# YuanchenBei/ColdRec

Hardware: AMD Instinct MI355X
Metric: ranked items/sec (full-catalogue eval) (higher is better)
Workload: dtype f32; 1 GPU; configs[3] full-catalogue eval: 1000000-row user table x 10000000 items, d=128, k=20, f32 tables, user block 131072 per step, rated CSR (mean ~50) + 20% cold-item bitmap ('warm' setting), item table row-sharded over 1 GPU(s); items=10000000, dim=128, k=20, parallelism=single GPU

## Files before the change

### coldrec_amd/_lib.py

```python
from __future__ import annotations

import ctypes
import os
import subprocess

_HERE = os.path.dirname(os.path.abspath(__file__))
LIB_PATH = os.environ.get("CRH_LIB") or os.path.join(_HERE, "lib", "libcoldrec_hip.so")
CSRC = os.path.join(_HERE, "csrc")

PAD_IDX = 0x7FFFFFFF
MASKED_SCORE = -1.0e9
MAX_K = 128

_lib = None

_vp, _i32, _i64, _sz, _f32 = ctypes.c_void_p, ctypes.c_int, ctypes.c_int64, ctypes.c_size_t, ctypes.c_float
_f64 = ctypes.c_double

SIGNATURES = {
    "crh_last_error": (ctypes.c_char_p, []),
    "crh_version": (_i32, []),
    "crh_score_topk_supports_dim": (_i32, [_i32]),
    "crh_score_topk_workspace_bytes": (_sz, [_i64, _i64, _i32, _i32]),
    "crh_score_topk_min_workspace_bytes": (_sz, [_i64, _i32]),
    "crh_score_topk_route": (_i32, [_i32, _i64, _i64, _i32, _i32, _sz, _i32, _i32, _vp, _vp]),
    "crh_score_topk_route_kernel": (ctypes.c_char_p, [_i32]),
    "crh_score_topk_screened": (_i32, [_i32, _i64, _i64, _i32, _i32, _sz, _i32, _i32]),
    "crh_score_topk_uncertified": (_i64, [_vp, _vp]),
    "crh_score_topk_screen_plan": (_i32, [_i64, _i64, _sz, _i32, _vp, _vp]),
    "crh_score_topk_screen_ordered": (_i32, [_i64, _i64, _sz, _i32]),
    "crh_score_topk_screen_map": (_i32, [_vp, _vp, _i64, _i64, _i64, _i32, _vp, _vp, _vp, _vp]),
    "crh_score_topk_f32": (_i32, [_vp, _vp, _i64, _vp, _i64, _i32, _vp, _vp, _vp, _i32, _i64, _vp, _vp,
                                  _vp, _sz, _vp]),
    "crh_score_topk_f32_ex": (_i32, [_vp, _vp, _i64, _vp, _i64, _i32, _vp, _vp, _vp, _i32, _i64, _vp, _vp,
                                     _vp, _sz, _vp, _i32, _vp, _vp]),
    "crh_score_topk_f16_supports_dim": (_i32, [_i32]),
    "crh_score_topk_f16_workspace_bytes": (_sz, [_i64, _i64, _i32, _i32]),
    "crh_score_topk_f16_ex": (_i32, [_vp, _vp, _i64, _vp, _i64, _i32, _vp, _vp, _vp, _i32, _i64, _vp, _vp,
                                     _vp, _sz, _vp, _i32, _vp, _vp]),
    "crh_mask_topk_f32": (_i32, [_vp, _i64, _i64, _i64, _vp, _vp, _vp, _i32, _i64, _i32, _vp, _vp, _vp]),
    "crh_merge_topk": (_i32, [_vp, _vp, _i32, _i64, _i32, _i32, _vp, _vp, _vp]),
    "crh_bpr_workspace_bytes": (_sz, [_i64]),
    "crh_bpr_plan_ints": (_i64, [_i64]),
    "crh_bpr_heavy_threshold": (_i32, []),
    "crh_bpr_plan_build_host": (_i32, [_vp, _vp, _vp, _i64, _i64, _vp]),
    "crh_bpr_plan_build": (_i32, [_vp, _vp, _vp, _i64, _i64, _vp, _vp]),
    "crh_bpr_plan_build_large_workspace_bytes": (_sz, [_i64, _i64]),
    "crh_bpr_plan_build_large": (_i32, [_vp, _vp, _vp, _i64, _i64, _vp, _vp, _sz, _vp]),
    "crh_bpr_fwd_bwd_f32": (_i32, [_vp, _vp, _vp, _i32, _vp, _vp, _vp, _i64, _f32, _vp, _vp, _vp, _vp, _vp, _vp,
                                   _sz, _vp]),
# ... 125 lines not shown
```

### coldrec_amd/csrc/score_screen.hip

```cpp
#include <math.h>

#include "score_topk_common.h"

#include <hipcub/device/device_radix_sort.hpp>

namespace crh_score {
namespace {

constexpr int SD = 128;
constexpr int FB_SCRATCH_SLICES = 64;

__device__ __forceinline__ float up_float(double x) {
    if (!(x <= 3.0e38)) return __builtin_inff();
    float f = (float)x;
    if ((double)f < x) f = __uint_as_float(__float_as_uint(f) + 1u);
    return f;
}

__device__ __forceinline__ int scale_exp(const unsigned* stats, int word) {
    const float m = __uint_as_float(stats[word]);
    if (!(m > 0.0f) || !(m <= 3.4e38f)) return 0;
    int E;
    frexpf(m, &E);
    return 15 - E;
// ... 453 lines not shown
    hipLaunchKernelGGL(screen_sortkey_kernel, dim3((unsigned)((n_slots + 255) / 256)), dim3(256), 0, st, idmap, ord->rowkeys, n_live,
                       item_base, n_slots, ord->skeys_in);
    CRH_HIP(hipGetLastError());
    size_t need = 0;
    CRH_HIP(hipcub::DeviceRadixSort::SortPairs(nullptr, need, ord->skeys_in, ord->skeys_out, idmap, ord->idmap, (int)n_slots, 0, 16, st));
    if (need > ord->sort_tmp_bytes) {
        crh_set_error("screened route: the ordered map's sort asks for %zu bytes of temporary storage, %zu are reserved", need,
                      ord->sort_tmp_bytes);
        return CRH_ERR_WS;
    }
    need = ord->sort_tmp_bytes;
    CRH_HIP(hipcub::DeviceRadixSort::SortPairs(ord->sort_tmp, need, ord->skeys_in, ord->skeys_out, idmap, ord->idmap, (int)n_slots, 0, 16, st));
    return CRH_OK;
}

int launch_screen_prep(const ScreenArgs& s, _Float16* packed, _Float16* uh, int64_t prefix, int32_t* idmap, unsigned* scan,
                       const ScreenOrder* ord, hipStream_t st) {
    const int64_t T = (s.n_items + 31) / 32;
    if (ord != nullptr)
        hipLaunchKernelGGL(screen_maxabs_kernel<true>, dim3(2048), dim3(256), 0, st, s.item_emb, nullptr, s.n_items, s.stats, 0, ord->rowkeys);
    else
        hipLaunchKernelGGL(screen_maxabs_kernel<false>, dim3(2048), dim3(256), 0, st, s.item_emb, nullptr, s.n_items, s.stats, 0, nullptr);
    CRH_HIP(hipGetLastError());
    hipLaunchKernelGGL(screen_maxabs_kernel<false>, dim3(256), dim3(256), 0, st, s.user_emb, s.users, s.n_users, s.stats, 1, nullptr);
    CRH_HIP(hipGetLastError());
    if (idmap != nullptr) {
        const int rc = launch_screen_map(s.bitmap, s.item_base, s.n_items, prefix, s.stats + SCREEN_STAT_LIVE, scan, idmap, ord, st);
        if (rc != CRH_OK) return rc;
        if (ord != nullptr) idmap = ord->idmap;
    }
    hipLaunchKernelGGL(screen_items_kernel, dim3((unsigned)(T < 4096 ? T : 4096)), dim3(256), 0, st, s.item_emb, s.n_items, s.bitmap,
                       s.item_base, packed, s.stats, prefix, idmap);
    CRH_HIP(hipGetLastError());
    const int64_t ub = (s.n_users * 16 + 255) / 256;
    hipLaunchKernelGGL(screen_users_kernel, dim3((unsigned)(ub < 2048 ? ub : 2048)), dim3(256), 0, st, s.user_emb, s.users, s.n_users,
                       uh, s.ustat, s.stats);
    CRH_HIP(hipGetLastError());
    return CRH_OK;
}

int screen_map_only(const uint32_t* bitmap, const float* item_emb, int64_t n_items, int64_t item_base, int64_t prefix, int ordered,
                    int32_t* map_out, int32_t* keys_out, int64_t* count, hipStream_t st) {
    auto al = [](size_t x) { return (x + 255) & ~(size_t)255; };
    const int64_t n_main = n_items - prefix, n_slots = screen_map_slots(n_main);
    const size_t o_scan = 256, o_map = o_scan + al(screen_scan_bytes(n_main)), o_rk = o_map + al((size_t)n_slots * 4),
                 o_k0 = o_rk + al((size_t)n_items * 2), o_k1 = o_k0 + al((size_t)n_slots * 2), o_m1 = o_k1 + al((size_t)n_slots * 2),
                 o_tmp = o_m1 + al((size_t)n_slots * 4), total = o_tmp + screen_sort_bytes(n_slots);
// ... 48 lines not shown
```

### coldrec_amd/csrc/score_topk.hip

```cpp
#include <math.h>
#include <stdarg.h>
#include <stdlib.h>

#include <algorithm>
#include <vector>

#include "score_topk_common.h"

using namespace crh_score;

namespace {

__device__ __forceinline__ bool pack_row_masked(const uint32_t* bitmap, int64_t gid) {
    return bitmap != nullptr && ((bitmap[gid >> 5] >> (gid & 31)) & 1u);
}

template <int D>
__global__ __launch_bounds__(256) void pack_items_kernel(const float* __restrict__ v, int64_t n_items,
                                                         float* __restrict__ packed, const uint32_t* __restrict__ bitmap,
                                                         int64_t item_base) {
    constexpr int NCH = D / 8;
    __shared__ float tile[32][D + 4];
    const int64_t t = blockIdx.x;
    for (int e = threadIdx.x; e < 32 * (D / 4); e += 256) {
// ... 810 lines not shown
    if (mode >= 2) return true;
    if (n_items < FP32_DMA_FLAG_MAX_ITEMS) return false;
    int64_t P = seed_route(esz, n_users, n_items, d);
    size_t ws = workspace_bytes;
    if (P > 0) {
        const size_t sb = seed_bytes(n_users, k);
        const size_t stage1 = dense_block_bytes(n_users, P) + packed_bytes(P, d, esz);
        const size_t stage2 = lists_bytes(n_users, k) + packed_bytes(n_items - P, d, esz);
        if (workspace_bytes >= sb + std::max(stage1, stage2)) ws = workspace_bytes - sb;
        else P = 0;
    }
    const RoutePlan r = plan_route(esz, n_users, n_items - P, d, k, true, ws, has_bitmap, 0, P > 0);
    return !r.dense && r.use_dma && r.dma_mode == 3;
}

int score_topk_screened(const float* user_emb, const int32_t* users, int64_t n_users, const float* item_emb, int64_t n_items,
                        const int64_t* rated_rowptr, const int32_t* rated_col, const uint32_t* cand_bitmap, int k, int64_t item_base,
                        float* out_score, int32_t* out_idx, void* workspace, size_t workspace_bytes, void* stream,
                        void* ev_kernel_start, void* ev_kernel_stop, const char* who);

int score_topk_any(int esz, const void* user_emb, const int32_t* users, int64_t n_users, const void* item_emb,
                   int64_t n_items, int d, const int64_t* rated_rowptr, const int32_t* rated_col,
                   const uint32_t* cand_bitmap, int k, int64_t item_base, float* out_score, int32_t* out_idx,
                   void* workspace, size_t workspace_bytes, void* stream, int n_splits, void* ev_kernel_start,
                   void* ev_kernel_stop, const char* who) {
    if (user_emb && item_emb && out_score && out_idx && workspace &&
        screen_route(esz, n_users, n_items, d, k, workspace_bytes, cand_bitmap != nullptr, n_splits))
        return score_topk_screened(reinterpret_cast<const float*>(user_emb), users, n_users, reinterpret_cast<const float*>(item_emb),
                                   n_items, rated_rowptr, rated_col, cand_bitmap, k, item_base, out_score, out_idx, workspace,
                                   workspace_bytes, stream, ev_kernel_start, ev_kernel_stop, who);
    const int64_t P = n_splits == 0 ? seed_route(esz, n_users, n_items, d) : 0;
    if (P > 0 && user_emb && item_emb && out_score && out_idx && n_users > 0 && k >= 1 && k <= CRH_MAX_K && workspace) {
        const size_t sb = seed_bytes(n_users, k);
        const size_t stage1 = dense_block_bytes(n_users, P) + packed_bytes(P, d, esz);
        const size_t stage2 = lists_bytes(n_users, k) + packed_bytes(n_items - P, d, esz);
        if (workspace_bytes >= sb + std::max(stage1, stage2)) {
            float* seed_s = reinterpret_cast<float*>(workspace);
            int32_t* seed_i = reinterpret_cast<int32_t*>(seed_s + (size_t)n_users * k);
            void* ws2 = reinterpret_cast<char*>(workspace) + sb;
            hipStream_t st = reinterpret_cast<hipStream_t>(stream);
            if (ev_kernel_start) CRH_HIP(hipEventRecord(reinterpret_cast<hipEvent_t>(ev_kernel_start), st));
            int rc = score_topk_impl(esz, user_emb, users, n_users, item_emb, P, d, rated_rowptr, rated_col, cand_bitmap, k,
                                     item_base, seed_s, seed_i, ws2, workspace_bytes - sb, stream, 0, nullptr, nullptr, who,
                                     nullptr, nullptr);
            if (rc != CRH_OK) return rc;
// ... 264 lines not shown
#ifdef CRH_PROFILE
    if (timing && use_dma) {
        rc = dma_timing_report(a, esz, d, st);
        if (rc != CRH_OK) return rc;
    }
    if (timing && !use_wg) {
        const int trc = print_wave_timing(a.wave_clock, n_waves, timing, st);
        if (trc != CRH_OK) return trc;
    }
#endif
    if (a.n_splits > 1)
        return crh_merge_topk(a.out_score, a.out_idx, a.n_splits, n_users, k, k, out_score, out_idx, stream);
    return CRH_OK;
}

int score_topk_screened(const float* user_emb, const int32_t* users, int64_t n_users, const float* item_emb, int64_t n_items,
                        const int64_t* rated_rowptr, const int32_t* rated_col, const uint32_t* cand_bitmap, int k, int64_t item_base,
                        float* out_score, int32_t* out_idx, void* workspace, size_t workspace_bytes, void* stream,
                        void* ev_kernel_start, void* ev_kernel_stop, const char* who) {
    CRH_CHECK_ARG(((uintptr_t)user_emb & 15) == 0 && ((uintptr_t)item_emb & 15) == 0, "%s: tables must be 16-byte aligned", who);
    CRH_CHECK_ARG(rated_rowptr != nullptr || rated_col == nullptr, "%s: rated_col given without rated_rowptr", who);
    CRH_CHECK_ARG(item_base >= 0 && item_base + n_items < (int64_t)CRH_PAD_IDX, "%s: item ids exceed int32", who);
    constexpr int KP = SCREEN_KP, D = 128;
    const int64_t P = screen_prefix(n_items);
    const bool compact = screen_compact(n_users, n_items, workspace_bytes, cand_bitmap != nullptr);
    const bool ordered = screen_ordered(n_users, n_items, workspace_bytes, cand_bitmap != nullptr);
    const ScreenLayout L = screen_layout(n_users, n_items, P, compact, ordered);
    CRH_CHECK_ARG(workspace_bytes >= L.need, "%s: workspace %zu < %zu bytes (screened route)", who, workspace_bytes, L.need);
    int32_t* idmap = compact ? reinterpret_cast<int32_t*>(reinterpret_cast<char*>(workspace) + L.idmap) : nullptr;
    hipStream_t st = reinterpret_cast<hipStream_t>(stream);
    char* ws = reinterpret_cast<char*>(workspace);
    ScreenOrder ord;
    if (ordered) {
        const size_t slots = (size_t)screen_map_slots(n_items - P);
        ord.rowkeys = reinterpret_cast<uint16_t*>(ws + L.rowkeys);
        ord.skeys_in = reinterpret_cast<uint16_t*>(ws + L.skeys);
        ord.skeys_out = reinterpret_cast<uint16_t*>(ws + L.skeys + (L.idmap2 - L.skeys) / 2);
        ord.idmap = reinterpret_cast<int32_t*>(ws + L.idmap2);
        ord.sort_tmp = ws + L.sorttmp;
        ord.sort_tmp_bytes = screen_sort_bytes((int64_t)slots);
    }
    _Float16* pk = reinterpret_cast<_Float16*>(ws + L.packed);
    _Float16* uh = reinterpret_cast<_Float16*>(ws + L.uh);
    float* seed_s = reinterpret_cast<float*>(ws + L.seed);
    int32_t* seed_i = reinterpret_cast<int32_t*>(seed_s + (size_t)n_users * KP);
    float* cand_s = reinterpret_cast<float*>(ws + L.cand);
    int32_t* cand_i = reinterpret_cast<int32_t*>(cand_s + (size_t)n_users * KP);
    char* scratch = ws + L.scratch;
    const size_t scratch_b = workspace_bytes - L.scratch;

    ScreenArgs s;
    s.user_emb = user_emb;
    s.users = users;
    s.n_users = n_users;
    s.item_emb = item_emb;
    s.n_items = n_items;
    s.item_base = item_base;
// ... 2 lines not shown
    s.bitmap = cand_bitmap;
    s.k = k;
    s.kp = KP;
    s.mode = screen_mode();
    s.cand_score = cand_s;
    s.cand_idx = cand_i;
    s.stats = reinterpret_cast<unsigned*>(ws + L.stats);
    s.ustat = reinterpret_cast<float*>(ws + L.ustat);
    s.fail_list = reinterpret_cast<int32_t*>(ws + L.fail);
    s.n_slices = screen_fallback_slices(n_items);
    s.part_score = reinterpret_cast<float*>(scratch);
    s.part_idx = reinterpret_cast<int32_t*>(s.part_score + (size_t)n_users * s.n_slices * k);
    s.out_score = out_score;
    s.out_idx = out_idx;

    CRH_HIP(hipMemsetAsync(s.stats, 0, 256, st));
    int rc = launch_screen_prep(s, pk, uh, P, idmap, reinterpret_cast<unsigned*>(ws + L.scan), ordered ? &ord : nullptr, st);
    if (rc != CRH_OK) return rc;
    if (ev_kernel_start) CRH_HIP(hipEventRecord(reinterpret_cast<hipEvent_t>(ev_kernel_start), st));

    ScoreArgs a;
    a.user_emb = uh;
    a.users = nullptr;
    a.n_users = n_users;
    a.item_emb = nullptr;
    a.rated_rowptr = rated_rowptr;
    a.rated_col = rated_col;
    a.bitmap = cand_bitmap;
    a.k = KP;
    a.ablate = 0;
    a.wave_clock = nullptr;
    a.xcd_sync = nullptr;
// ... 52 lines not shown
        a.out_score = reinterpret_cast<float*>(scratch);
        a.out_idx = reinterpret_cast<int32_t*>(a.out_score + (size_t)a.n_splits * n_users * KP);
    }
    static const int sync_win_raw = CRH_TUNE_ENV("CRH_SCORE_SYNC_WINDOW") ? atoi(CRH_TUNE_ENV("CRH_SCORE_SYNC_WINDOW")) : 128;
    static const int sync_win = sync_win_raw <= 0 ? 0 : std::max(2, sync_win_raw & ~1);
    if (sync_win > 0 && a.n_splits == 1 && n_wg <= 256 && n_wg > 8) {
        const int64_t n_win = (T + 1 + sync_win - 1) / sync_win + 1;
        if ((size_t)(n_win + 1) * 8 * sizeof(unsigned) <= sync_bytes(n_items)) {
            a.sync_window = sync_win;
            a.sync_stride = n_win + 1;
            a.xcd_sync = reinterpret_cast<unsigned*>(ws + L.sync);
            CRH_HIP(hipMemsetAsync(a.xcd_sync, 0, (size_t)a.sync_stride * 8 * sizeof(unsigned), st));
        }
    }
    if (compact) {
        a.idmap = ordered ? ord.idmap : idmap;
        a.n_live = s.stats + SCREEN_STAT_LIVE;
    } else if (cand_bitmap) {
        uint32_t* tb = reinterpret_cast<uint32_t*>(ws + L.tbits);
        hipLaunchKernelGGL(tile_bits_kernel, dim3((unsigned)((T + 255) / 256)), dim3(256), 0, st, cand_bitmap, a.item_base, n_main, T, tb);
        CRH_HIP(hipGetLastError());
        a.tile_bits = tb;
    }
#ifdef CRH_PROFILE
    static const int timing = CRH_PROFILE_ENV("CRH_SCORE_TIMING");
    if (timing) {
        rc = dma_timing_begin(a, st);
        if (rc != CRH_OK) return rc;
    }
#endif
    rc = launch_score_dma(2, D, 3, a, st);
    if (rc != CRH_OK) return rc;
#ifdef CRH_PROFILE
    if (timing) {
        rc = dma_timing_report(a, 2, D, st);
        if (rc != CRH_OK) return rc;
    }
// ... 83 lines not shown
    return screen_ordered(n_users, n_items, workspace_bytes, has_bitmap != 0) ? 1 : 0;
}

extern "C" int crh_score_topk_screen_map(const uint32_t* bitmap, const float* item_emb, int64_t n_items, int64_t item_base,
                                         int64_t prefix, int ordered, int32_t* map_out, int32_t* keys_out, int64_t* count,
                                         void* stream) {
    CRH_CHECK_ARG(bitmap && item_emb && map_out && keys_out && count, "crh_score_topk_screen_map: NULL argument");
    CRH_CHECK_ARG(prefix >= 0 && (prefix & 31) == 0 && n_items > prefix, "crh_score_topk_screen_map: prefix %lld of %lld items",
                  (long long)prefix, (long long)n_items);
    CRH_CHECK_ARG(((uintptr_t)item_emb & 15) == 0, "crh_score_topk_screen_map: table must be 16-byte aligned");
    CRH_CHECK_ARG(item_base >= 0 && item_base + n_items < (int64_t)CRH_PAD_IDX, "crh_score_topk_screen_map: item ids exceed int32");
    return screen_map_only(bitmap, item_emb, n_items, item_base, prefix, ordered, map_out, keys_out, count,
                           reinterpret_cast<hipStream_t>(stream));
}

extern "C" int64_t crh_score_topk_uncertified(const void* workspace, void* stream) {
    CRH_CHECK_ARG(workspace != nullptr, "crh_score_topk_uncertified: NULL workspace");
    unsigned n = 0;
    hipStream_t st = reinterpret_cast<hipStream_t>(stream);
    CRH_HIP(hipMemcpyAsync(&n, reinterpret_cast<const unsigned*>(workspace) + 5, sizeof(n), hipMemcpyDeviceToHost, st));
    CRH_HIP(hipStreamSynchronize(st));
    return (int64_t)n;
}

extern "C" const char* crh_score_topk_route_kernel(int route) {
    switch (route & 15) {
        case CRH_ROUTE_DENSE: return "score_topk_kernel";
        case CRH_ROUTE_FUSED_WAVE: return "score_topk_kernel";
        case CRH_ROUTE_FUSED_WG: return "score_topk_wg_kernel";
        case CRH_ROUTE_FUSED_DMA: return "score_topk_dma_kernel";
// ... 1 lines not shown
    }
}

extern "C" int crh_score_topk_f32_ex(const float* user_emb, const int32_t* users, int64_t n_users,
                                     const float* item_emb, int64_t n_items, int d,
                                     const int64_t* rated_rowptr, const int32_t* rated_col,
                                     const uint32_t* cand_bitmap, int k, int64_t item_base,
                                     float* out_score, int32_t* out_idx, void* workspace,
                                     size_t workspace_bytes, void* stream, int n_splits,
                                     void* ev_kernel_start, void* ev_kernel_stop) {
    return score_topk_any(4, user_emb, users, n_users, item_emb, n_items, d, rated_rowptr, rated_col, cand_bitmap, k,
                          item_base, out_score, out_idx, workspace, workspace_bytes, stream, n_splits,
                          ev_kernel_start, ev_kernel_stop, "crh_score_topk_f32");
}

extern "C" int crh_score_topk_f32(const float* user_emb, const int32_t* users, int64_t n_users,
                                  const float* item_emb, int64_t n_items, int d,
                                  const int64_t* rated_rowptr, const int32_t* rated_col,
                                  const uint32_t* cand_bitmap, int k, int64_t item_base,
                                  float* out_score, int32_t* out_idx, void* workspace,
                                  size_t workspace_bytes, void* stream) {
    return crh_score_topk_f32_ex(user_emb, users, n_users, item_emb, n_items, d, rated_rowptr, rated_col,
                                 cand_bitmap, k, item_base, out_score, out_idx, workspace, workspace_bytes,
                                 stream, 0, nullptr, nullptr);
}

extern "C" int crh_score_topk_f16_ex(const void* user_emb, const int32_t* users, int64_t n_users,
                                     const void* item_emb, int64_t n_items, int d,
                                     const int64_t* rated_rowptr, const int32_t* rated_col,
                                     const uint32_t* cand_bitmap, int k, int64_t item_base,
// ... 8 lines not shown
```

### coldrec_amd/csrc/score_topk_common.h

```cpp
#pragma once
#include <math.h>

#include "crh_common.h"
#include "topk_list.h"

namespace crh_score {

struct ScoreArgs {
    const void* user_emb;
    const int32_t* users;
    int64_t n_users;
    const void* item_emb;
    const void* packed;
    int64_t n_items;
    const int64_t* rated_rowptr;
    const int32_t* rated_col;
    const uint32_t* bitmap;
    int k;
    int64_t item_base;
    int n_splits;
    int64_t n_ugroups;
    float* out_score;
    int32_t* out_idx;
    int ablate;
// ... 318 lines not shown
    int32_t* out_idx;
};
__attribute__((visibility("hidden"))) int screen_fallback_slices(int64_t n_items);
constexpr int SCREEN_STAT_LIVE = 6;
__attribute__((visibility("hidden"))) size_t screen_scan_bytes(int64_t n_main);
struct ScreenOrder {
    uint16_t* rowkeys;
    uint16_t* skeys_in;
    uint16_t* skeys_out;
    int32_t* idmap;
    void* sort_tmp;
    size_t sort_tmp_bytes;
};
__attribute__((visibility("hidden"))) int64_t screen_map_slots(int64_t n_main);
__attribute__((visibility("hidden"))) size_t screen_sort_bytes(int64_t n_slots);
__attribute__((visibility("hidden"))) int launch_screen_prep(const ScreenArgs& s, _Float16* packed, _Float16* uh, int64_t prefix,
                                                             int32_t* idmap, unsigned* scan, const ScreenOrder* ord, hipStream_t st);
__attribute__((visibility("hidden"))) int screen_map_only(const uint32_t* bitmap, const float* item_emb, int64_t n_items,
                                                          int64_t item_base, int64_t prefix, int ordered, int32_t* map_out,
                                                          int32_t* keys_out, int64_t* count, hipStream_t st);
__attribute__((visibility("hidden"))) int launch_screen_certify(const ScreenArgs& s, hipStream_t st);

}
```

### coldrec_amd/eval.py

```python
from __future__ import annotations

import os
from typing import Tuple

import torch

from . import ops


def shard_bounds(n_items: int, world: int, rank: int) -> Tuple[int, int]:
    return rank * n_items // world, (rank + 1) * n_items // world


class UserShardedTopK:

    def __init__(self, items: torch.Tensor, k: int, world: int = 1, rank: int = 0, group=None):
        self.items, self.k = items, int(k)
        self.world, self.rank, self.group = world, rank, group

    def topk(self, user_emb, users, rated_rowptr=None, rated_col=None, cand_bitmap=None):
        n = users.shape[0]
        lo, hi = self.rank * n // self.world, (self.rank + 1) * n // self.world
        rp = rc = None
        if rated_rowptr is not None:
            rp = (rated_rowptr[lo:hi + 1] - rated_rowptr[lo]).contiguous()
            rc = rated_col[int(rated_rowptr[lo]):int(rated_rowptr[hi])].contiguous()
        s, i = ops.score_topk(user_emb, users[lo:hi].contiguous(), self.items, self.k, rp, rc, cand_bitmap)
        if self.world == 1:
            return s, i
        import torch.distributed as dist
        longest = (n + self.world - 1) // self.world
        packed = torch.zeros((longest, 2 * self.k), dtype=torch.int32, device=s.device)
        packed[: hi - lo] = torch.cat([s.view(torch.int32), i], dim=1)
        flat = torch.empty((self.world * longest, 2 * self.k), dtype=torch.int32, device=s.device)
        dist.all_gather_into_tensor(flat, packed, group=self.group)
        rows = [flat[r * longest: r * longest + ((r + 1) * n // self.world - r * n // self.world)]
                for r in range(self.world)]
        full = torch.cat(rows, 0)
        return full[:, : self.k].contiguous().view(torch.float32), full[:, self.k:].contiguous()


class ShardedTopK:
    def __init__(self, item_shard: torch.Tensor, item_base: int, n_items_global: int, k: int,
                 world: int = 1, rank: int = 0, group=None):
        self.items = item_shard
        self.item_base = int(item_base)
        self.n_items_global = int(n_items_global)
        self.k = int(k)
        self.world, self.rank, self.group = world, rank, group
        self.force_collective = bool(int(os.environ.get("CRH_FORCE_COLLECTIVE", "0")))

    def topk(self, user_emb, users, rated_rowptr=None, rated_col=None, cand_bitmap=None, n_splits: int = 0,
             kernel_events=None):
        kw = {}
        if kernel_events is not None:
            kw["kernel_events"] = kernel_events
        if n_splits:
            kw["n_splits"] = n_splits
        s, i = ops.score_topk(user_emb, users, self.items, self.k, rated_rowptr, rated_col, cand_bitmap,
                              item_base=self.item_base, **kw)
        if self.world == 1 and not self.force_collective:
            return s, i
        import torch.distributed as dist
        packed = torch.cat([s.view(torch.int32), i], dim=1).contiguous()
        flat = torch.empty((self.world * packed.shape[0], packed.shape[1]), dtype=torch.int32,
                           device=packed.device)
        dist.all_gather_into_tensor(flat, packed, group=self.group)
        gathered = flat.view(self.world, packed.shape[0], packed.shape[1])
        gs = gathered[:, :, :self.k].contiguous().view(torch.float32)
        gi = gathered[:, :, self.k:].contiguous()
        return ops.merge_topk(gs, gi, self.k)
```

### coldrec_amd/ops.py

```python
from __future__ import annotations

import ctypes
import weakref
import os
from typing import Optional, Tuple

import numpy as np
import torch

from . import _lib

SUPPORTED_DIMS = (8, 16, 32, 64, 128, 256)
SUPPORTED_DIMS_F16 = (16, 32, 64, 128, 256)


def _need_cuda(*ts):
    for t in ts:
        if t is not None and not t.is_cuda:
            raise RuntimeError("coldrec_amd ops need tensors on the MI355X (cuda device); there is no CPU path")


def pad_dim(table: torch.Tensor) -> torch.Tensor:
    d = table.shape[1]
    dims = SUPPORTED_DIMS_F16 if table.dtype == torch.float16 else SUPPORTED_DIMS
# ... 33 lines not shown
_ws_cache = {}


def _workspace(nbytes: int, device) -> torch.Tensor:
    key = (device.type, device.index, torch.cuda.current_stream(device).cuda_stream)
    buf = _ws_cache.get(key)
    if buf is None or buf.numel() < nbytes:
        buf = torch.empty(max(nbytes, 1 << 20), dtype=torch.uint8, device=device)
        _ws_cache[key] = buf
    return buf


def score_topk(user_emb: torch.Tensor, users: Optional[torch.Tensor], item_emb: torch.Tensor, k: int,
               rated_rowptr: Optional[torch.Tensor] = None, rated_col: Optional[torch.Tensor] = None,
               cand_bitmap: Optional[torch.Tensor] = None, item_base: int = 0, n_splits: int = 0,
               out: Optional[Tuple[torch.Tensor, torch.Tensor]] = None, kernel_events=None, pack: bool = True):
    _need_cuda(user_emb, users, item_emb, rated_rowptr, rated_col, cand_bitmap)
    if user_emb.dtype != item_emb.dtype or user_emb.dtype not in (torch.float32, torch.float16):
        raise RuntimeError("score_topk: both tables fp32 (exact, canonical) or both fp16 (fp32 accumulate)")
    half = user_emb.dtype == torch.float16
    if user_emb.shape[1] != item_emb.shape[1]:
        raise RuntimeError("score_topk: user/item embedding widths differ")
    user_emb, item_emb = pad_dim(user_emb.contiguous()), pad_dim(item_emb.contiguous())
    if users is not None:
        users = users.to(torch.int32).contiguous()
    n_users = user_emb.shape[0] if users is None else users.shape[0]
    n_items, d = item_emb.shape
    if rated_rowptr is not None:
        assert rated_rowptr.dtype == torch.int64 and rated_col.dtype == torch.int32
        assert rated_rowptr.shape[0] == n_users + 1
    if cand_bitmap is not None:
        assert cand_bitmap.dtype == torch.int32
    dev = user_emb.device
    if out is None:
        out = (torch.empty((n_users, k), dtype=torch.float32, device=dev),
               torch.empty((n_users, k), dtype=torch.int32, device=dev))
    L = _lib.lib()
    full = L.crh_score_topk_f16_workspace_bytes if half else L.crh_score_topk_workspace_bytes
    ws_bytes = full(n_users, n_items, d, k) if pack else L.crh_score_topk_min_workspace_bytes(n_users, k)
    ws = _workspace(ws_bytes, dev)
    rc = (L.crh_score_topk_f16_ex if half else L.crh_score_topk_f32_ex)(_lib.ptr(user_emb), _lib.ptr(users), n_users, _lib.ptr(item_emb), n_items, d,
                                 _lib.ptr(rated_rowptr), _lib.ptr(rated_col), _lib.ptr(cand_bitmap), k,
                                 item_base, _lib.ptr(out[0]), _lib.ptr(out[1]), _lib.ptr(ws), ws_bytes,
                                 _lib.current_stream(), n_splits,
                                 kernel_events[0] if kernel_events else None,
                                 kernel_events[1] if kernel_events else None)
    _lib.check(rc, "crh_score_topk_f32")
    return out


ROUTE_NAMES = {1: "dense", 2: "fused-wave", 3: "fused-wg", 4: "fused-dma"}


def score_topk_route(n_users: int, n_items: int, d: int, k: int, half: bool = False, has_bitmap: bool = True,
                     n_splits: int = 0, pack: bool = True) -> dict:
    import ctypes
    L = _lib.lib()
    d = d if d % 8 == 0 and (L.crh_score_topk_f16_supports_dim(d) if half else L.crh_score_topk_supports_dim(d)) else \
        next(w for w in (8, 16, 32, 64, 128, 256) if w >= d and (w >= 16 or not half))
    full = L.crh_score_topk_f16_workspace_bytes if half else L.crh_score_topk_workspace_bytes
    ws_bytes = full(n_users, n_items, d, k) if pack else L.crh_score_topk_min_workspace_bytes(n_users, k)
    prefix, splits = ctypes.c_int64(0), ctypes.c_int(0)
    code = L.crh_score_topk_route(2 if half else 4, n_users, n_items, d, k, ws_bytes, 1 if has_bitmap else 0, n_splits,
# ... 779 lines not shown
```

### include/coldrec_hip.h

```cpp
#ifndef COLDREC_HIP_H
#define COLDREC_HIP_H

#include <stddef.h>
#include <stdint.h>

#ifdef __cplusplus
extern "C" {
#endif

#define CRH_OK 0
#define CRH_ERR_ARG (-1)
#define CRH_ERR_HIP (-2)
#define CRH_ERR_WS (-3)
#define CRH_PAD_IDX 0x7fffffff
#define CRH_MASKED_SCORE (-1.0e9f)
#define CRH_MAX_K 128

const char* crh_last_error(void);
int crh_version(void);
int crh_score_topk_supports_dim(int d);

size_t crh_score_topk_workspace_bytes(int64_t n_users, int64_t n_items, int d, int k);
size_t crh_score_topk_min_workspace_bytes(int64_t n_users, int k);

// ... 1 lines not shown
#define CRH_ROUTE_FUSED_WAVE 2
#define CRH_ROUTE_FUSED_WG 3
#define CRH_ROUTE_FUSED_DMA 4
#define CRH_ROUTE_SEEDED 16
#define CRH_ROUTE_DMA_FLAGS 32
int crh_score_topk_route(int elem_bytes, int64_t n_users, int64_t n_items, int d, int k, size_t workspace_bytes,
                         int has_bitmap, int n_splits, int64_t* prefix_items, int* picked_splits);
const char* crh_score_topk_route_kernel(int route);
int crh_score_topk_screen_plan(int64_t n_users, int64_t n_items, size_t workspace_bytes, int has_bitmap, int* cuts, int* compact);
int crh_score_topk_screen_ordered(int64_t n_users, int64_t n_items, size_t workspace_bytes, int has_bitmap);
int crh_score_topk_screen_map(const uint32_t* bitmap, const float* item_emb, int64_t n_items, int64_t item_base, int64_t prefix,
                              int ordered, int32_t* map_out, int32_t* keys_out, int64_t* count, void* stream);
int crh_score_topk_screened(int elem_bytes, int64_t n_users, int64_t n_items, int d, int k, size_t workspace_bytes,
                            int has_bitmap, int n_splits);
int64_t crh_score_topk_uncertified(const void* workspace, void* stream);
int crh_score_topk_f32(const float* user_emb, const int32_t* users, int64_t n_users,
                       const float* item_emb, int64_t n_items, int d,
                       const int64_t* rated_rowptr, const int32_t* rated_col,
                       const uint32_t* cand_bitmap, int k, int64_t item_base,
                       float* out_score, int32_t* out_idx,
                       void* workspace, size_t workspace_bytes, void* stream);

int crh_score_topk_f32_ex(const float* user_emb, const int32_t* users, int64_t n_users,
                          const float* item_emb, int64_t n_items, int d,
                          const int64_t* rated_rowptr, const int32_t* rated_col,
                          const uint32_t* cand_bitmap, int k, int64_t item_base,
                          float* out_score, int32_t* out_idx,
                          void* workspace, size_t workspace_bytes, void* stream, int n_splits,
                          void* ev_kernel_start, void* ev_kernel_stop);

// ... 205 lines not shown
```

Baseline: 5978 billion items/s.

## Cache screened item-side prep across user blocks via a prepared-items handle

Splits screen prep into an item half (max-abs stats, fp16 packing, live-item map/sort, tile bits) and a user half. Adds a PreparedItems object that builds the item half once into its own buffer. Later calls that match on table pointer, version, bitmap, base and stream only copy the stats and rerun the user prep. This avoids re-reading and re-packing the 10M-item table for every 131072-user block. The cost is a persistent extra buffer and a validity check that relies on tensor pointers and version counters.

```diff
diff --git a/coldrec_amd/_lib.py b/coldrec_amd/_lib.py
--- a/coldrec_amd/_lib.py
+++ b/coldrec_amd/_lib.py
@@ -34,6 +34,12 @@
                                   _vp, _sz, _vp]),
     "crh_score_topk_f32_ex": (_i32, [_vp, _vp, _i64, _vp, _i64, _i32, _vp, _vp, _vp, _i32, _i64, _vp, _vp,
                                      _vp, _sz, _vp, _i32, _vp, _vp]),
+    "crh_score_screen_items_bytes": (_sz, [_i64, _i32]),
+    "crh_score_screen_items_prepare": (_i32, [_vp, _i64, _i32, _vp, _i64, _i64, _vp, _sz, _vp, _sz, _vp, _vp]),
+    "crh_score_screen_items_destroy": (_i32, [_vp]),
+    "crh_score_topk_screen_item_preps": (_i64, []),
+    "crh_score_topk_f32_prepared": (_i32, [_vp, _vp, _i64, _vp, _i64, _i32, _vp, _vp, _vp, _i32, _i64, _vp, _vp,
+                                           _vp, _sz, _vp, _i32, _vp, _vp, _vp]),
     "crh_score_topk_f16_supports_dim": (_i32, [_i32]),
     "crh_score_topk_f16_workspace_bytes": (_sz, [_i64, _i64, _i32, _i32]),
     "crh_score_topk_f16_ex": (_i32, [_vp, _vp, _i64, _vp, _i64, _i32, _vp, _vp, _vp, _i32, _i64, _vp, _vp,
diff --git a/coldrec_amd/csrc/score_screen.hip b/coldrec_amd/csrc/score_screen.hip
--- a/coldrec_amd/csrc/score_screen.hip
+++ b/coldrec_amd/csrc/score_screen.hip
@@ -491,23 +491,27 @@
     return CRH_OK;
 }
 
-int launch_screen_prep(const ScreenArgs& s, _Float16* packed, _Float16* uh, int64_t prefix, int32_t* idmap, unsigned* scan,
-                       const ScreenOrder* ord, hipStream_t st) {
+int launch_screen_prep_items(const ScreenArgs& s, unsigned* stats, _Float16* packed, int64_t prefix, int32_t* idmap, unsigned* scan,
+                             const ScreenOrder* ord, hipStream_t st) {
     const int64_t T = (s.n_items + 31) / 32;
     if (ord != nullptr)
-        hipLaunchKernelGGL(screen_maxabs_kernel<true>, dim3(2048), dim3(256), 0, st, s.item_emb, nullptr, s.n_items, s.stats, 0, ord->rowkeys);
+        hipLaunchKernelGGL(screen_maxabs_kernel<true>, dim3(2048), dim3(256), 0, st, s.item_emb, nullptr, s.n_items, stats, 0, ord->rowkeys);
     else
-        hipLaunchKernelGGL(screen_maxabs_kernel<false>, dim3(2048), dim3(256), 0, st, s.item_emb, nullptr, s.n_items, s.stats, 0, nullptr);
-    CRH_HIP(hipGetLastError());
-    hipLaunchKernelGGL(screen_maxabs_kernel<false>, dim3(256), dim3(256), 0, st, s.user_emb, s.users, s.n_users, s.stats, 1, nullptr);
+        hipLaunchKernelGGL(screen_maxabs_kernel<false>, dim3(2048), dim3(256), 0, st, s.item_emb, nullptr, s.n_items, stats, 0, nullptr);
     CRH_HIP(hipGetLastError());
     if (idmap != nullptr) {
-        const int rc = launch_screen_map(s.bitmap, s.item_base, s.n_items, prefix, s.stats + SCREEN_STAT_LIVE, scan, idmap, ord, st);
+        const int rc = launch_screen_map(s.bitmap, s.item_base, s.n_items, prefix, stats + SCREEN_STAT_LIVE, scan, idmap, ord, st);
         if (rc != CRH_OK) return rc;
         if (ord != nullptr) idmap = ord->idmap;
     }
     hipLaunchKernelGGL(screen_items_kernel, dim3((unsigned)(T < 4096 ? T : 4096)), dim3(256), 0, st, s.item_emb, s.n_items, s.bitmap,
-                       s.item_base, packed, s.stats, prefix, idmap);
+                       s.item_base, packed, stats, prefix, idmap);
+    CRH_HIP(hipGetLastError());
+    return CRH_OK;
+}
+
+int launch_screen_prep_users(const ScreenArgs& s, _Float16* uh, hipStream_t st) {
+    hipLaunchKernelGGL(screen_maxabs_kernel<false>, dim3(256), dim3(256), 0, st, s.user_emb, s.users, s.n_users, s.stats, 1, nullptr);
     CRH_HIP(hipGetLastError());
     const int64_t ub = (s.n_users * 16 + 255) / 256;
     hipLaunchKernelGGL(screen_users_kernel, dim3((unsigned)(ub < 2048 ? ub : 2048)), dim3(256), 0, st, s.user_emb, s.users, s.n_users,
diff --git a/coldrec_amd/csrc/score_topk.hip b/coldrec_amd/csrc/score_topk.hip
--- a/coldrec_amd/csrc/score_topk.hip
+++ b/coldrec_amd/csrc/score_topk.hip
@@ -3,6 +3,7 @@
 #include <stdlib.h>
 
 #include <algorithm>
+#include <atomic>
 #include <vector>
 
 #include "score_topk_common.h"
@@ -848,21 +849,55 @@
     return !r.dense && r.use_dma && r.dma_mode == 3;
 }
 
+constexpr uint32_t SCREEN_ITEMS_MAGIC = 0x43524849u;
+struct ScreenItems {
+    uint32_t magic;
+    const float* item_emb;
+    int64_t n_items, item_base, prefix;
+    int d;
+    const uint32_t* bitmap;
+    bool compact, ordered;
+    hipStream_t stream;
+    char* buf;
+};
+struct ScreenItemsLayout {
+    size_t stats, packed, tbits, map, need;
+};
+ScreenItemsLayout screen_items_layout(int64_t n_items, bool has_bitmap) {
+    ScreenItemsLayout L;
+    L.stats = 0;
+    L.packed = 256;
+    L.tbits = L.packed + packed_bytes(n_items, 128, 2);
+    L.map = L.tbits + (has_bitmap ? tbits_bytes(n_items) : 0);
+    const size_t slots = (size_t)screen_map_slots(n_items);
+    L.need = L.map + (has_bitmap ? (slots * sizeof(int32_t) + 255) & ~(size_t)255 : 0);
+    return L;
+}
+bool screen_items_match(const ScreenItems* p, const float* item_emb, int64_t n_items, int64_t item_base, const uint32_t* bitmap,
+                        int64_t prefix, bool compact, bool ordered, hipStream_t st) {
+    if (p == nullptr || p->magic != SCREEN_ITEMS_MAGIC) return false;
+    const char* e = getenv("CRH_SCORE_SCREEN_PREPARED");
+    if (e && atoi(e) == 0) return false;
+    return p->item_emb == item_emb && p->n_items == n_items && p->d == 128 && p->item_base == item_base && p->bitmap == bitmap &&
+           p->prefix == prefix && p->compact == compact && p->ordered == ordered && p->stream == st;
+}
+std::atomic<int64_t> screen_item_preps{0};
+
 int score_topk_screened(const float* user_emb, const int32_t* users, int64_t n_users, const float* item_emb, int64_t n_items,
                         const int64_t* rated_rowptr, const int32_t* rated_col, const uint32_t* cand_bitmap, int k, int64_t item_base,
                         float* out_score, int32_t* out_idx, void* workspace, size_t workspace_bytes, void* stream,
-                        void* ev_kernel_start, void* ev_kernel_stop, const char* who);
+                        void* ev_kernel_start, void* ev_kernel_stop, const char* who, const ScreenItems* prepared);
 
 int score_topk_any(int esz, const void* user_emb, const int32_t* users, int64_t n_users, const void* item_emb,
                    int64_t n_items, int d, const int64_t* rated_rowptr, const int32_t* rated_col,
                    const uint32_t* cand_bitmap, int k, int64_t item_base, float* out_score, int32_t* out_idx,
                    void* workspace, size_t workspace_bytes, void* stream, int n_splits, void* ev_kernel_start,
-                   void* ev_kernel_stop, const char* who) {
+                   void* ev_kernel_stop, const char* who, const ScreenItems* prepared = nullptr) {
     if (user_emb && item_emb && out_score && out_idx && workspace &&
         screen_route(esz, n_users, n_items, d, k, workspace_bytes, cand_bitmap != nullptr, n_splits))
         return score_topk_screened(reinterpret_cast<const float*>(user_emb), users, n_users, reinterpret_cast<const float*>(item_emb),
                                    n_items, rated_rowptr, rated_col, cand_bitmap, k, item_base, out_score, out_idx, workspace,
-                                   workspace_bytes, stream, ev_kernel_start, ev_kernel_stop, who);
+                                   workspace_bytes, stream, ev_kernel_start, ev_kernel_stop, who, prepared);
     const int64_t P = n_splits == 0 ? seed_route(esz, n_users, n_items, d) : 0;
     if (P > 0 && user_emb && item_emb && out_score && out_idx && n_users > 0 && k >= 1 && k <= CRH_MAX_K && workspace) {
         const size_t sb = seed_bytes(n_users, k);
@@ -1157,10 +1192,23 @@
     return CRH_OK;
 }
 
+int screen_items_build(const ScreenArgs& s, unsigned* stats, _Float16* pk, int64_t P, int32_t* idmap, unsigned* scan,
+                       const ScreenOrder* ord, uint32_t* tbits, hipStream_t st) {
+    screen_item_preps.fetch_add(1, std::memory_order_relaxed);
+    const int rc = launch_screen_prep_items(s, stats, pk, P, idmap, scan, ord, st);
+    if (rc != CRH_OK) return rc;
+    if (tbits != nullptr) {
+        const int64_t n_main = s.n_items - P, T = (n_main + 31) / 32;
+        hipLaunchKernelGGL(tile_bits_kernel, dim3((unsigned)((T + 255) / 256)), dim3(256), 0, st, s.bitmap, s.item_base + P, n_main, T, tbits);
+        CRH_HIP(hipGetLastError());
+    }
+    return CRH_OK;
+}
+
 int score_topk_screened(const float* user_emb, const int32_t* users, int64_t n_users, const float* item_emb, int64_t n_items,
                         const int64_t* rated_rowptr, const int32_t* rated_col, const uint32_t* cand_bitmap, int k, int64_t item_base,
                         float* out_score, int32_t* out_idx, void* workspace, size_t workspace_bytes, void* stream,
-                        void* ev_kernel_start, void* ev_kernel_stop, const char* who) {
+                        void* ev_kernel_start, void* ev_kernel_stop, const char* who, const ScreenItems* prepared) {
     CRH_CHECK_ARG(((uintptr_t)user_emb & 15) == 0 && ((uintptr_t)item_emb & 15) == 0, "%s: tables must be 16-byte aligned", who);
     CRH_CHECK_ARG(rated_rowptr != nullptr || rated_col == nullptr, "%s: rated_col given without rated_rowptr", who);
     CRH_CHECK_ARG(item_base >= 0 && item_base + n_items < (int64_t)CRH_PAD_IDX, "%s: item ids exceed int32", who);
@@ -1183,7 +1231,12 @@
         ord.sort_tmp = ws + L.sorttmp;
         ord.sort_tmp_bytes = screen_sort_bytes((int64_t)slots);
     }
-    _Float16* pk = reinterpret_cast<_Float16*>(ws + L.packed);
+    const bool reuse = screen_items_match(prepared, item_emb, n_items, item_base, cand_bitmap, P, compact, ordered, st);
+    const ScreenItemsLayout PL = screen_items_layout(n_items, cand_bitmap != nullptr);
+    _Float16* pk = reinterpret_cast<_Float16*>(reuse ? prepared->buf + PL.packed : ws + L.packed);
+    uint32_t* tbits = cand_bitmap && !compact ? reinterpret_cast<uint32_t*>(reuse ? prepared->buf + PL.tbits : ws + L.tbits) : nullptr;
+    const int32_t* stream_map = nullptr;
+    if (compact) stream_map = reuse ? reinterpret_cast<const int32_t*>(prepared->buf + PL.map) : (ordered ? ord.idmap : idmap);
     _Float16* uh = reinterpret_cast<_Float16*>(ws + L.uh);
     float* seed_s = reinterpret_cast<float*>(ws + L.seed);
     int32_t* seed_i = reinterpret_cast<int32_t*>(seed_s + (size_t)n_users * KP);
@@ -1216,8 +1269,15 @@
     s.out_score = out_score;
     s.out_idx = out_idx;
 
-    CRH_HIP(hipMemsetAsync(s.stats, 0, 256, st));
-    int rc = launch_screen_prep(s, pk, uh, P, idmap, reinterpret_cast<unsigned*>(ws + L.scan), ordered ? &ord : nullptr, st);
+    int rc = CRH_OK;
+    if (reuse) {
+        CRH_HIP(hipMemcpyAsync(s.stats, prepared->buf + PL.stats, 256, hipMemcpyDeviceToDevice, st));
+    } else {
+        CRH_HIP(hipMemsetAsync(s.stats, 0, 256, st));
+        rc = screen_items_build(s, s.stats, pk, P, idmap, reinterpret_cast<unsigned*>(ws + L.scan), ordered ? &ord : nullptr, tbits, st);
+        if (rc != CRH_OK) return rc;
+    }
+    rc = launch_screen_prep_users(s, uh, st);
     if (rc != CRH_OK) return rc;
     if (ev_kernel_start) CRH_HIP(hipEventRecord(reinterpret_cast<hipEvent_t>(ev_kernel_start), st));
 
@@ -1300,13 +1360,10 @@
         }
     }
     if (compact) {
-        a.idmap = ordered ? ord.idmap : idmap;
+        a.idmap = stream_map;
         a.n_live = s.stats + SCREEN_STAT_LIVE;
     } else if (cand_bitmap) {
-        uint32_t* tb = reinterpret_cast<uint32_t*>(ws + L.tbits);
-        hipLaunchKernelGGL(tile_bits_kernel, dim3((unsigned)((T + 255) / 256)), dim3(256), 0, st, cand_bitmap, a.item_base, n_main, T, tb);
-        CRH_HIP(hipGetLastError());
-        a.tile_bits = tb;
+        a.tile_bits = tbits;
     }
 #ifdef CRH_PROFILE
     static const int timing = CRH_PROFILE_ENV("CRH_SCORE_TIMING");
@@ -1420,6 +1477,80 @@
                            reinterpret_cast<hipStream_t>(stream));
 }
 
+extern "C" size_t crh_score_screen_items_bytes(int64_t n_items, int has_bitmap) {
+    if (n_items <= 0) return 0;
+    return screen_items_layout(n_items, has_bitmap != 0).need;
+}
+
+extern "C" int crh_score_screen_items_prepare(const float* item_emb, int64_t n_items, int d, const uint32_t* cand_bitmap,
+                                              int64_t item_base, int64_t n_users, void* items_buf, size_t items_bytes,
+                                              void* workspace, size_t workspace_bytes, void* stream, void** handle) {
+    const char* who = "crh_score_screen_items_prepare";
+    CRH_CHECK_ARG(item_emb && items_buf && workspace && handle, "%s: NULL argument", who);
+    CRH_CHECK_ARG(d == 128, "%s: d=%d (the screened route ranks d=128 tables)", who, d);
+    CRH_CHECK_ARG(n_users > 0 && n_items > 0, "%s: empty block", who);
+    CRH_CHECK_ARG(((uintptr_t)item_emb & 15) == 0 && ((uintptr_t)items_buf & 255) == 0, "%s: table must be 16-byte, buffer 256-byte aligned", who);
+    CRH_CHECK_ARG(item_base >= 0 && item_base + n_items < (int64_t)CRH_PAD_IDX, "%s: item ids exceed int32", who);
+    const bool has_bitmap = cand_bitmap != nullptr;
+    const ScreenItemsLayout PL = screen_items_layout(n_items, has_bitmap);
+    CRH_CHECK_ARG(items_bytes >= PL.need, "%s: buffer %zu < %zu bytes", who, items_bytes, PL.need);
+    const int64_t P = screen_prefix(n_items);
+    const bool compact = screen_compact(n_users, n_items, workspace_bytes, has_bitmap);
+    const bool ordered = screen_ordered(n_users, n_items, workspace_bytes, has_bitmap);
+    const ScreenLayout L = screen_layout(n_users, n_items, P, compact, ordered);
+    CRH_CHECK_ARG(workspace_bytes >= L.need, "%s: workspace %zu < %zu bytes (screened route)", who, workspace_bytes, L.need);
+    hipStream_t st = reinterpret_cast<hipStream_t>(stream);
+    char* ws = reinterpret_cast<char*>(workspace);
+    char* buf = reinterpret_cast<char*>(items_buf);
+    int32_t* own_map = reinterpret_cast<int32_t*>(buf + PL.map);
+    ScreenOrder ord;
+    if (ordered) {
+        const size_t slots = (size_t)screen_map_slots(n_items - P);
+        ord.rowkeys = reinterpret_cast<uint16_t*>(ws + L.rowkeys);
+        ord.skeys_in = reinterpret_cast<uint16_t*>(ws + L.skeys);
+        ord.skeys_out = reinterpret_cast<uint16_t*>(ws + L.skeys + (L.idmap2 - L.skeys) / 2);
+        ord.idmap = own_map;
+        ord.sort_tmp = ws + L.sorttmp;
+        ord.sort_tmp_bytes = screen_sort_bytes((int64_t)slots);
+    }
+    int32_t* idmap = compact ? (ordered ? reinterpret_cast<int32_t*>(ws + L.idmap) : own_map) : nullptr;
+    ScreenArgs s = {};
+    s.item_emb = item_emb;
+    s.n_items = n_items;
+    s.item_base = item_base;
+    s.bitmap = cand_bitmap;
+    unsigned* stats = reinterpret_cast<unsigned*>(buf + PL.stats);
+    CRH_HIP(hipMemsetAsync(stats, 0, 256, st));
+    const int rc = screen_items_build(s, stats, reinterpret_cast<_Float16*>(buf + PL.packed), P, idmap, reinterpret_cast<unsigned*>(ws + L.scan),
+                                      ordered ? &ord : nullptr, has_bitmap && !compact ? reinterpret_cast<uint32_t*>(buf + PL.tbits) : nullptr, st);
+    if (rc != CRH_OK) return rc;
+    ScreenItems* p = new ScreenItems;
+    p->magic = SCREEN_ITEMS_MAGIC;
+    p->item_emb = item_emb;
+    p->n_items = n_items;
+    p->item_base = item_base;
+    p->prefix = P;
+    p->d = d;
+    p->bitmap = cand_bitmap;
+    p->compact = compact;
+    p->ordered = ordered;
+    p->stream = st;
+    p->buf = buf;
+    *handle = p;
+    return CRH_OK;
+}
+
+extern "C" int crh_score_screen_items_destroy(void* handle) {
+    if (handle == nullptr) return CRH_OK;
+    ScreenItems* p = reinterpret_cast<ScreenItems*>(handle);
+    CRH_CHECK_ARG(p->magic == SCREEN_ITEMS_MAGIC, "crh_score_screen_items_destroy: not a prepared-items handle");
+    p->magic = 0;
+    delete p;
+    return CRH_OK;
+}
+
+extern "C" int64_t crh_score_topk_screen_item_preps(void) { return screen_item_preps.load(std::memory_order_relaxed); }
+
 extern "C" int64_t crh_score_topk_uncertified(const void* workspace, void* stream) {
     CRH_CHECK_ARG(workspace != nullptr, "crh_score_topk_uncertified: NULL workspace");
     unsigned n = 0;
@@ -1451,6 +1582,18 @@
                           ev_kernel_start, ev_kernel_stop, "crh_score_topk_f32");
 }
 
+extern "C" int crh_score_topk_f32_prepared(const float* user_emb, const int32_t* users, int64_t n_users,
+                                           const float* item_emb, int64_t n_items, int d,
+                                           const int64_t* rated_rowptr, const int32_t* rated_col,
+                                           const uint32_t* cand_bitmap, int k, int64_t item_base,
+                                           float* out_score, int32_t* out_idx, void* workspace,
+                                           size_t workspace_bytes, void* stream, int n_splits,
+                                           void* ev_kernel_start, void* ev_kernel_stop, const void* prepared) {
+    return score_topk_any(4, user_emb, users, n_users, item_emb, n_items, d, rated_rowptr, rated_col, cand_bitmap, k,
+                          item_base, out_score, out_idx, workspace, workspace_bytes, stream, n_splits,
+                          ev_kernel_start, ev_kernel_stop, "crh_score_topk_f32", reinterpret_cast<const ScreenItems*>(prepared));
+}
+
 extern "C" int crh_score_topk_f32(const float* user_emb, const int32_t* users, int64_t n_users,
                                   const float* item_emb, int64_t n_items, int d,
                                   const int64_t* rated_rowptr, const int32_t* rated_col,
diff --git a/coldrec_amd/csrc/score_topk_common.h b/coldrec_amd/csrc/score_topk_common.h
--- a/coldrec_amd/csrc/score_topk_common.h
+++ b/coldrec_amd/csrc/score_topk_common.h
@@ -356,8 +356,9 @@
 };
 __attribute__((visibility("hidden"))) int64_t screen_map_slots(int64_t n_main);
 __attribute__((visibility("hidden"))) size_t screen_sort_bytes(int64_t n_slots);
-__attribute__((visibility("hidden"))) int launch_screen_prep(const ScreenArgs& s, _Float16* packed, _Float16* uh, int64_t prefix,
-                                                             int32_t* idmap, unsigned* scan, const ScreenOrder* ord, hipStream_t st);
+__attribute__((visibility("hidden"))) int launch_screen_prep_items(const ScreenArgs& s, unsigned* stats, _Float16* packed, int64_t prefix,
+                                                                   int32_t* idmap, unsigned* scan, const ScreenOrder* ord, hipStream_t st);
+__attribute__((visibility("hidden"))) int launch_screen_prep_users(const ScreenArgs& s, _Float16* uh, hipStream_t st);
 __attribute__((visibility("hidden"))) int screen_map_only(const uint32_t* bitmap, const float* item_emb, int64_t n_items,
                                                           int64_t item_base, int64_t prefix, int ordered, int32_t* map_out,
                                                           int32_t* keys_out, int64_t* count, hipStream_t st);
diff --git a/coldrec_amd/eval.py b/coldrec_amd/eval.py
--- a/coldrec_amd/eval.py
+++ b/coldrec_amd/eval.py
@@ -12,7 +12,31 @@
     return rank * n_items // world, (rank + 1) * n_items // world
 
 
-class UserShardedTopK:
+class _PreparedShard:
+
+    def _prepared(self, n_users: int, cand_bitmap, item_base: int, n_splits: int = 0):
+        items = self.items
+        if not items.is_cuda or items.dtype != torch.float32 or items.dim() != 2 or items.shape[1] != 128 or not items.is_contiguous():
+            return None
+        if cand_bitmap is not None and not cand_bitmap.is_contiguous():
+            return None
+        if not ops.score_topk_route(n_users, items.shape[0], 128, self.k, has_bitmap=cand_bitmap is not None,
+                                    n_splits=n_splits)["screened"]:
+            return None
+        prep = getattr(self, "_prep", None)
+        if prep is None or not prep.fits(items, cand_bitmap, item_base):
+            self._prep = prep = None
+            try:
+                self._prep = prep = ops.prepare_items(items, cand_bitmap, item_base)
+            except torch.cuda.OutOfMemoryError:
+                return None
+        return prep
+
+    def refresh(self) -> None:
+        self._prep = None
+
+
+class UserShardedTopK(_PreparedShard):
 
     def __init__(self, items: torch.Tensor, k: int, world: int = 1, rank: int = 0, group=None):
         self.items, self.k = items, int(k)
@@ -25,7 +49,9 @@
         if rated_rowptr is not None:
             rp = (rated_rowptr[lo:hi + 1] - rated_rowptr[lo]).contiguous()
             rc = rated_col[int(rated_rowptr[lo]):int(rated_rowptr[hi])].contiguous()
-        s, i = ops.score_topk(user_emb, users[lo:hi].contiguous(), self.items, self.k, rp, rc, cand_bitmap)
+        prep = self._prepared(hi - lo, cand_bitmap, 0)
+        s, i = ops.score_topk(user_emb, users[lo:hi].contiguous(), self.items, self.k, rp, rc, cand_bitmap,
+                              **({} if prep is None else {"prepared": prep}))
         if self.world == 1:
             return s, i
         import torch.distributed as dist
@@ -40,7 +66,8 @@
         return full[:, : self.k].contiguous().view(torch.float32), full[:, self.k:].contiguous()
 
 
-class ShardedTopK:
+class ShardedTopK(_PreparedShard):
+
     def __init__(self, item_shard: torch.Tensor, item_base: int, n_items_global: int, k: int,
                  world: int = 1, rank: int = 0, group=None):
         self.items = item_shard
@@ -57,6 +84,9 @@
             kw["kernel_events"] = kernel_events
         if n_splits:
             kw["n_splits"] = n_splits
+        prep = self._prepared(user_emb.shape[0] if users is None else users.shape[0], cand_bitmap, self.item_base, n_splits)
+        if prep is not None:
+            kw["prepared"] = prep
         s, i = ops.score_topk(user_emb, users, self.items, self.k, rated_rowptr, rated_col, cand_bitmap,
                               item_base=self.item_base, **kw)
         if self.world == 1 and not self.force_collective:
diff --git a/coldrec_amd/ops.py b/coldrec_amd/ops.py
--- a/coldrec_amd/ops.py
+++ b/coldrec_amd/ops.py
@@ -71,7 +71,8 @@
 def score_topk(user_emb: torch.Tensor, users: Optional[torch.Tensor], item_emb: torch.Tensor, k: int,
                rated_rowptr: Optional[torch.Tensor] = None, rated_col: Optional[torch.Tensor] = None,
                cand_bitmap: Optional[torch.Tensor] = None, item_base: int = 0, n_splits: int = 0,
-               out: Optional[Tuple[torch.Tensor, torch.Tensor]] = None, kernel_events=None, pack: bool = True):
+               out: Optional[Tuple[torch.Tensor, torch.Tensor]] = None, kernel_events=None, pack: bool = True,
+               prepared: Optional["PreparedItems"] = None):
     _need_cuda(user_emb, users, item_emb, rated_rowptr, rated_col, cand_bitmap)
     if user_emb.dtype != item_emb.dtype or user_emb.dtype not in (torch.float32, torch.float16):
         raise RuntimeError("score_topk: both tables fp32 (exact, canonical) or both fp16 (fp32 accumulate)")
@@ -96,14 +97,84 @@
     full = L.crh_score_topk_f16_workspace_bytes if half else L.crh_score_topk_workspace_bytes
     ws_bytes = full(n_users, n_items, d, k) if pack else L.crh_score_topk_min_workspace_bytes(n_users, k)
     ws = _workspace(ws_bytes, dev)
-    rc = (L.crh_score_topk_f16_ex if half else L.crh_score_topk_f32_ex)(_lib.ptr(user_emb), _lib.ptr(users), n_users, _lib.ptr(item_emb), n_items, d,
-                                 _lib.ptr(rated_rowptr), _lib.ptr(rated_col), _lib.ptr(cand_bitmap), k,
-                                 item_base, _lib.ptr(out[0]), _lib.ptr(out[1]), _lib.ptr(ws), ws_bytes,
-                                 _lib.current_stream(), n_splits,
-                                 kernel_events[0] if kernel_events else None,
-                                 kernel_events[1] if kernel_events else None)
+    args = (_lib.ptr(user_emb), _lib.ptr(users), n_users, _lib.ptr(item_emb), n_items, d,
+            _lib.ptr(rated_rowptr), _lib.ptr(rated_col), _lib.ptr(cand_bitmap), k,
+            item_base, _lib.ptr(out[0]), _lib.ptr(out[1]), _lib.ptr(ws), ws_bytes,
+            _lib.current_stream(), n_splits,
+            kernel_events[0] if kernel_events else None,
+            kernel_events[1] if kernel_events else None)
+    if prepared is not None and not half and pack and prepared.fits(item_emb, cand_bitmap, item_base):
+        rc = L.crh_score_topk_f32_prepared(*args, prepared.handle_for(n_users, ws, ws_bytes))
+    else:
+        rc = (L.crh_score_topk_f16_ex if half else L.crh_score_topk_f32_ex)(*args)
     _lib.check(rc, "crh_score_topk_f32")
     return out
+
+
+class PreparedItems:
+
+    def __init__(self, item_emb: torch.Tensor, cand_bitmap: Optional[torch.Tensor] = None, item_base: int = 0):
+        _need_cuda(item_emb, cand_bitmap)
+        if item_emb.dtype != torch.float32 or item_emb.dim() != 2 or item_emb.shape[1] != 128 or not item_emb.is_contiguous():
+            raise RuntimeError("prepare_items: the screened route ranks contiguous fp32 tables of width 128")
+        if cand_bitmap is not None and (cand_bitmap.dtype != torch.int32 or not cand_bitmap.is_contiguous()):
+            raise RuntimeError("prepare_items: cand_bitmap must be contiguous int32 words")
+        self.item_emb, self.cand_bitmap, self.item_base = item_emb, cand_bitmap, int(item_base)
+        self.item_ptr, self.item_version = item_emb.data_ptr(), item_emb._version
+        self.bitmap_ptr = None if cand_bitmap is None else cand_bitmap.data_ptr()
+        self.bitmap_version = None if cand_bitmap is None else cand_bitmap._version
+        self.stream = torch.cuda.current_stream(item_emb.device).cuda_stream
+        nbytes = int(_lib.lib().crh_score_screen_items_bytes(item_emb.shape[0], 0 if cand_bitmap is None else 1))
+        self.buf = torch.empty(max(nbytes, 1), dtype=torch.uint8, device=item_emb.device)
+        self.handle = None
+
+    def fits(self, item_emb: torch.Tensor, cand_bitmap: Optional[torch.Tensor], item_base: int = 0) -> bool:
+        if item_emb.data_ptr() != self.item_ptr or item_emb.shape != self.item_emb.shape or int(item_base) != self.item_base:
+            return False
+        if self.item_emb._version != self.item_version or item_emb._version != self.item_version:
+            return False
+        if (cand_bitmap is None) != (self.cand_bitmap is None):
+            return False
+        if cand_bitmap is not None and (cand_bitmap.data_ptr() != self.bitmap_ptr or cand_bitmap._version != self.bitmap_version
+                                        or self.cand_bitmap._version != self.bitmap_version):
+            return False
+        return torch.cuda.current_stream(item_emb.device).cuda_stream == self.stream
+
+    def handle_for(self, n_users: int, ws: torch.Tensor, ws_bytes: int):
+        if self.handle is None:
+            h = ctypes.c_void_p(None)
+            rc = _lib.lib().crh_score_screen_items_prepare(self.item_ptr, self.item_emb.shape[0], 128, self.bitmap_ptr, self.item_base,
+                                                           int(n_users), _lib.ptr(self.buf), self.buf.numel(), _lib.ptr(ws),
+                                                           int(ws_bytes), self.stream, ctypes.byref(h))
+            _lib.check(rc, "crh_score_screen_items_prepare")
+            self.handle = h
+        return self.handle
+
+    def build(self, n_users: int, k: int) -> "PreparedItems":
+        if torch.cuda.current_stream(self.item_emb.device).cuda_stream != self.stream:
+            raise RuntimeError("PreparedItems.build: not the stream the state was made on")
+        ws_bytes = int(_lib.lib().crh_score_topk_workspace_bytes(int(n_users), self.item_emb.shape[0], 128, int(k)))
+        self.handle_for(n_users, _workspace(ws_bytes, self.item_emb.device), ws_bytes)
+        return self
+
+    def close(self) -> None:
+        h, self.handle = self.handle, None
+        if h is not None:
+            _lib.lib().crh_score_screen_items_destroy(h)
+
+    def __del__(self):
+        try:
+            self.close()
+        except Exception:
+            pass
+
+
+def prepare_items(item_emb: torch.Tensor, cand_bitmap: Optional[torch.Tensor] = None, item_base: int = 0) -> PreparedItems:
+    return PreparedItems(item_emb, cand_bitmap, item_base)
+
+
+def screen_item_preps() -> int:
+    return int(_lib.lib().crh_score_topk_screen_item_preps())
 
 
 ROUTE_NAMES = {1: "dense", 2: "fused-wave", 3: "fused-wg", 4: "fused-dma"}
diff --git a/include/coldrec_hip.h b/include/coldrec_hip.h
--- a/include/coldrec_hip.h
+++ b/include/coldrec_hip.h
@@ -39,6 +39,19 @@
 int crh_score_topk_screened(int elem_bytes, int64_t n_users, int64_t n_items, int d, int k, size_t workspace_bytes,
                             int has_bitmap, int n_splits);
 int64_t crh_score_topk_uncertified(const void* workspace, void* stream);
+size_t crh_score_screen_items_bytes(int64_t n_items, int has_bitmap);
+int crh_score_screen_items_prepare(const float* item_emb, int64_t n_items, int d, const uint32_t* cand_bitmap, int64_t item_base,
+                                   int64_t n_users, void* items_buf, size_t items_bytes, void* workspace, size_t workspace_bytes,
+                                   void* stream, void** handle);
+int crh_score_screen_items_destroy(void* handle);
+int64_t crh_score_topk_screen_item_preps(void);
+int crh_score_topk_f32_prepared(const float* user_emb, const int32_t* users, int64_t n_users,
+                                const float* item_emb, int64_t n_items, int d,
+                                const int64_t* rated_rowptr, const int32_t* rated_col,
+                                const uint32_t* cand_bitmap, int k, int64_t item_base,
+                                float* out_score, int32_t* out_idx, void* workspace,
+                                size_t workspace_bytes, void* stream, int n_splits,
+                                void* ev_kernel_start, void* ev_kernel_stop, const void* prepared);
 int crh_score_topk_f32(const float* user_emb, const int32_t* users, int64_t n_users,
                        const float* item_emb, int64_t n_items, int d,
                        const int64_t* rated_rowptr, const int32_t* rated_col,
```

New measurement: 6059 billion items/s (median of 6 runs). 1.4% higher.
